# sisl/MADRL

Hardware: AMD Instinct MI355X
Metric: env-steps/sec at fixed batch (PursuitEvade 16x16, 8v30) (higher is better)
Workload: dtype u8/int32 grid state, f32 observations, f64 reward arithmetic; 1 GPU; PursuitEvade 16x16, 8 pursuers / 30 evaders, obs_range 7, rectangle_map, surround, n_catch 2, flatten, local reward, 65536 envs per GPU, horizon 500; envs_per_gpu=65536, envs_total=65536, parallelism=env-sharded x1, streams_per_gpu=2, rccl_ranks=1

## Files before the change

### madrl_amd/csrc/pursuit_wave.hpp

```cpp
#pragma once

#include <type_traits>

#include "common.hpp"

namespace madrl {
namespace pw {

#ifndef MADRL_PW_WAVES
#define MADRL_PW_WAVES 5
#endif
#define MADRL_PW_OCC __attribute__((amdgpu_waves_per_eu(S::OCC, S::OCC)))

constexpr uint32_t SENT = 0xFFFFFFFFu;
constexpr uint32_t CAUGHT = 0x10000u;

struct WaveDev {
    int32_t n_catch, surround, reward_global, sample_maps, n_maps, max_steps, auto_reset;
    int32_t fmap_stride;
    int32_t max_opponents;
    int32_t reverse;
    uint32_t k0, k1, gid_base;
    double catchr, term_pursuit, urgency, cw;
    int64_t n_envs;
    const uint32_t *fmaps;
    const float *vtab;
    const int32_t *pending;
    const uint32_t *cnt_tmpl;
    const uint32_t *slot_tab;
    const double *cw_env;
    const double *catchr_env;
    uint8_t *state;
    uint32_t *flags;
    uint32_t *zmask;
};

struct WaveIO {
    const uint8_t *mask;
    const int32_t *inj_pos;
    const int32_t *inj_map;
    const int32_t *actions;
    const int32_t *inj_eact;
    float *obs;
    float *rew;
    uint8_t *done;
    int32_t *removed;
    int32_t flex;
    int32_t control_evaders;
    const float *obs_prev;
};

__device__ __forceinline__ double sload_f64(const double *p, int64_t index) {
    return ((const __attribute__((address_space(4))) double *)(uint64_t)p)[index];
}

struct KArgs {
    WaveDev d;
    WaveIO io;
};
typedef const __attribute__((address_space(4))) KArgs *KArgsPtr;
__device__ __forceinline__ KArgsPtr cold_args() { return kernargs<KArgs>(); }
__device__ __forceinline__ int32_t pending_count(int64_t env, int k) {
    const int32_t *pend = cold_args()->d.pending;
    return ((const __attribute__((address_space(4))) int32_t *)(uint64_t)pend)[2 * env + k];
}

template <int XS_, int YS_, int P_, int E_, int R_, int FLATTEN_>
struct Shape {
    static constexpr int XS = XS_, YS = YS_, P = P_, E = E_, A = P_ + E_, R = R_, FLATTEN = FLATTEN_;
    static constexpr int OFF = (R - 1) / 2;
    static constexpr int PAD = OFF > 1 ? OFF : 1;
    static constexpr int GW = YS + 2 * PAD;
    static constexpr int GH = XS + 2 * PAD;
    static constexpr int GSZ = (GH * GW + 3) / 4 * 4;
    static constexpr int D = FLATTEN ? 3 * R * R + 1 : 4 * R * R;
    static constexpr int DV = D / 4;
    static constexpr int NQ = P * DV;
    static constexpr int NS = (NQ + 63) / 64;
    static constexpr int MWORDS = 1;
    static constexpr int OCC = NS <= 5 ? MADRL_PW_WAVES : (MADRL_PW_WAVES < 4 ? MADRL_PW_WAVES : 4);
    static constexpr int X_FILL = 3 * GSZ;
    static constexpr int X_SKIP = 3 * GSZ + 1;
    static constexpr int X_ID = 3 * GSZ + 2;
    static constexpr int X_VTAB = (X_ID + P + 3) / 4 * 4;
    static constexpr int NVT = 72;
    static constexpr int X_NEED = X_VTAB + NVT;
    static constexpr int X_OBSV = X_NEED + (XS * YS + 3) / 4;
    static constexpr int LDS_DWORDS = X_OBSV + (P + 3) / 4 * 4;
    static constexpr int NGW = (E + 31) / 32 > 0 ? (E + 31) / 32 : 1;
    static constexpr int NTW = (A + 31) / 32;
    static constexpr int OFF_GONE = (16 + 2 * A + 3) / 4 * 4;
    static constexpr int OFF_TERM = OFF_GONE + 4 * NGW;
    static constexpr int REC_BYTES = (OFF_TERM + 4 * NTW + 15) / 16 * 16;
    static constexpr int REC_DW = REC_BYTES / 4;
    static_assert(REC_DW <= 64, "the whole record must fit one dword per lane");
    static_assert(A <= 64, "one wavefront per env: n_pursuers + n_evaders must fit 64 lanes");
    static_assert(R % 2 == 1, "odd obs_range only (even ranges run on the generic kernel)");
    static_assert(D % 4 == 0, "observation row must be a whole number of float4");
    static_assert(LDS_DWORDS * 4 <= 64 * 1024, "LDS budget");
    static_assert(NS <= 8, "stale-zero mask: one bit per slot in each byte of the lane's mask dword");
    static constexpr bool LIVE = false;
    static constexpr bool TO = false;
    static constexpr bool TABLED = false;
    static constexpr int X_TAB = 0;
};

template <int XS_, int YS_, int P_, int E_, int R_, int FLATTEN_>
struct LShape : Shape<XS_, YS_, P_, E_, R_, FLATTEN_> {
    static constexpr bool LIVE = true;
};
constexpr int NOT_HERE = 0xFF;

template <int XS_, int YS_, int P_, int E_, int R_, int FLATTEN_>
struct TShape : Shape<XS_, YS_, P_, E_, R_, FLATTEN_> {
    static constexpr bool TO = true;
};
template <int XS_, int YS_, int P_, int E_, int R_, int FLATTEN_>
struct TLShape : LShape<XS_, YS_, P_, E_, R_, FLATTEN_> {
    static constexpr bool TO = true;
};

__device__ __forceinline__ double pairwise8(const double *r) {
    return ((r[0] + r[1]) + (r[2] + r[3])) + ((r[4] + r[5]) + (r[6] + r[7]));
}

template <int P>
__device__ __forceinline__ double np_sum_regs(const double (&a)[P]) {
    if constexpr (P < 8) {
        double res = 0.0;
#pragma unroll
        for (int i = 0; i < P; ++i) res += a[i];
        return res;
    } else {
        double r[8];
#pragma unroll
        for (int i = 0; i < 8; ++i) r[i] = a[i];
        constexpr int LIM = P - (P % 8);
#pragma unroll
        for (int i = 8; i < LIM; i += 8) {
#pragma unroll
            for (int k = 0; k < 8; ++k) r[k] += a[i + k];
        }
        double res = pairwise8(r);
#pragma unroll
        for (int i = LIM; i < P; ++i) res += a[i];
        return res;
    }
}

template <int P>
__device__ __forceinline__ double np_sum_first(const double (&a)[P], int n) {
    double res = 0.0;
    if (n < 8) {
#pragma unroll
        for (int i = 0; i < (P < 8 ? P : 7); ++i)
            if (i < n) res += a[i];
        return res;
    }
    if constexpr (P >= 8) {
        double r[8];
#pragma unroll
        for (int i = 0; i < 8; ++i) r[i] = a[i];
        const int lim = n - (n % 8);
#pragma unroll
        for (int i = 8; i + 8 <= P; i += 8) {
            if (i < lim) {
#pragma unroll
                for (int k = 0; k < 8; ++k) r[k] += a[i + k];
            }
        }
        res = pairwise8(r);
#pragma unroll
        for (int i = 8; i < P; ++i)
            if (i >= lim && i < n) res += a[i];
    }
    return res;
}

typedef float v4f_t __attribute__((ext_vector_type(4)));
template <int I, int N, class F>
__device__ __forceinline__ void static_for(F &&f) {
    if constexpr (I < N) {
        f(std::integral_constant<int, I>{});
        static_for<I + 1, N>(f);
    }
}
template <int OFF>
__device__ __forceinline__ void store_slot_masked(const void *base, uint32_t voff, uint32_t v0, uint32_t v1, uint32_t v2, uint32_t v3,
                                                  v4f_t val, uint64_t m0, uint64_t m1, uint64_t m2, uint64_t m3, uint64_t m_nt) {
    uint64_t sv;
    asm volatile("s_mov_b64 %0, exec\n\t"
                 "s_mov_b64 exec, %1\n\tglobal_store_dword %6, %7, %12 offset:%13\n\t"
                 "s_mov_b64 exec, %2\n\tglobal_store_dword %6, %8, %12 offset:%13+4\n\t"
                 "s_mov_b64 exec, %3\n\tglobal_store_dword %6, %9, %12 offset:%13+8\n\t"
                 "s_mov_b64 exec, %4\n\tglobal_store_dword %6, %10, %12 offset:%13+12\n\t"
                 "s_mov_b64 exec, %5\n\tglobal_store_dwordx4 %6, %11, %12 offset:%13 nt\n\t"
                 "s_mov_b64 exec, %0\n\ts_nop 0"
                 : "=&s"(sv) : "s"(m0), "s"(m1), "s"(m2), "s"(m3), "s"(m_nt), "v"(voff), "v"(v0), "v"(v1), "v"(v2), "v"(v3), "v"(val),
                   "s"(base), "n"(OFF));
}
__device__ __forceinline__ uint32_t quad_or(uint32_t v) {
    v |= (uint32_t)__builtin_amdgcn_update_dpp(0, (int)v, 0xB1, 0xF, 0xF, true);
    v |= (uint32_t)__builtin_amdgcn_update_dpp(0, (int)v, 0x4E, 0xF, 0xF, true);
    return v;
}

__device__ __forceinline__ void prefetch3(uint32_t &r0, uint32_t &r1, uint32_t &r2, const void *b0, uint32_t o0, const void *b1, uint32_t o1,
                                          const void *b2, uint32_t o2) {
    asm volatile("s_nop 4\n\tglobal_load_dword %0, %3, %4\n\tglobal_load_dword %1, %5, %6\n\tglobal_load_dword %2, %7, %8"
                 : "=&v"(r0), "=&v"(r1), "=&v"(r2) : "v"(o0), "s"(b0), "v"(o1), "s"(b1), "v"(o2), "s"(b2));
}
template <int N>
__device__ __forceinline__ void prefetch_wait(uint32_t &r0, uint32_t &r1, uint32_t &r2) {
    static_assert(N >= 0 && N < 64, "vmcnt is a 6-bit field");
    asm volatile("s_waitcnt vmcnt(%3)" : "+v"(r0), "+v"(r1), "+v"(r2) : "n"(N) : "memory");
}

template <int LN>
__device__ __forceinline__ void put_lane(uint32_t &w, uint32_t v) {
    const uint32_t sv = (uint32_t)__builtin_amdgcn_readfirstlane((int)v);
    asm("v_writelane_b32 %0, %1, %2" : "+v"(w) : "s"(sv), "n"(LN));
}
template <int LN, int END>
__device__ __forceinline__ void put_zero_from(uint32_t &w) {
    if constexpr (LN < END) {
        put_lane<LN>(w, 0u);
        put_zero_from<LN + 1, END>(w);
    }
}

template <class S, int NT>
struct Fill {
    static constexpr int NEEDW = (S::XS * S::YS + 3) / 4;
    static constexpr int TABW = S::TABLED ? 2 * S::DV : 0;
    static constexpr int J_MAP = (S::GSZ + NT - 1) / NT;
    static constexpr int J_NEED = 2 * J_MAP;
    static constexpr int J_VT = J_NEED + (NEEDW + NT - 1) / NT;
    static constexpr int J_TAB = J_VT + (S::NVT + NT - 1) / NT;
    static constexpr int J_END = J_TAB + (TABW + NT - 1) / NT;
    static constexpr int first(int j) { return j < J_MAP ? 0 : j < J_NEED ? J_MAP : j < J_VT ? J_NEED : j < J_TAB ? J_VT : J_TAB; }
    static constexpr int words(int j) { return j < J_NEED ? S::GSZ : j < J_VT ? NEEDW : j < J_TAB ? S::NVT : TABW; }
};
template <class S, int NT, int J>
__device__ __forceinline__ uint32_t fill_load(uint32_t utid, const uint32_t *cnt, const uint32_t *map, const uint32_t *vtab, const uint32_t *tab) {
    using F = Fill<S, NT>;
    constexpr int t = J - F::first(J), n = F::words(J);
    const uint32_t k = utid + (uint32_t)(NT * t);
    const uint32_t kc = (NT * (t + 1) <= n) ? k : (k < (uint32_t)n ? k : (uint32_t)n - 1u);
    if constexpr (J < F::J_MAP) return cnt[kc];
    else if constexpr (J < F::J_NEED) return map[kc];
    else if constexpr (J < F::J_VT) return map[(uint32_t)S::GSZ + kc];
    else if constexpr (J < F::J_TAB) return vtab[kc];
    else return tab[kc];
}
template <class S, int NT, int J, bool FIRST>
__device__ __forceinline__ void fill_store(uint32_t *L, uint32_t utid, uint32_t v) {
    using F = Fill<S, NT>;
    constexpr int t = J - F::first(J), n = F::words(J);
    const uint32_t k = utid + (uint32_t)(NT * t);
    if ((NT * (t + 1) <= n) || k < (uint32_t)n) {
        if constexpr (J < F::J_MAP) {
            L[S::GSZ + k] = v;
            L[2 * S::GSZ + k] = v;
        } else if constexpr (J < F::J_NEED) L[k] = v;
        else if constexpr (J < F::J_VT) L[S::X_NEED + k] = v;
        else if constexpr (J < F::J_TAB) L[S::X_VTAB + k] = v;
        else L[S::X_TAB + k] = v;
    }
    if constexpr (FIRST && J == F::J_MAP) {
        if (utid == 0u) {
            L[S::X_FILL] = v;
            L[S::X_SKIP] = SENT;
        }
    }
}
template <int N>
__device__ __forceinline__ void staged_wait(uint32_t *a) {
    if constexpr (N >= 8) {
        asm volatile("" : "+v"(a[N - 1]), "+v"(a[N - 2]), "+v"(a[N - 3]), "+v"(a[N - 4]), "+v"(a[N - 5]), "+v"(a[N - 6]), "+v"(a[N - 7]), "+v"(a[N - 8]));
        staged_wait<N - 8>(a);
    } else if constexpr (N >= 4) {
        asm volatile("" : "+v"(a[N - 1]), "+v"(a[N - 2]), "+v"(a[N - 3]), "+v"(a[N - 4]));
        staged_wait<N - 4>(a);
    } else if constexpr (N >= 2) {
        asm volatile("" : "+v"(a[N - 1]), "+v"(a[N - 2]));
        staged_wait<N - 2>(a);
    } else if constexpr (N == 1) {
        asm volatile("" : "+v"(a[0]));
    }
}
template <class S, int NT, int J0, int J1, int CAP, bool FIRST>
__device__ __forceinline__ void fill_trips(uint32_t *L, uint32_t utid, const uint32_t *cnt, const uint32_t *map, const uint32_t *vtab, const uint32_t *tab) {
    if constexpr (J0 < J1) {
        constexpr int JB = J0 + CAP < J1 ? J0 + CAP : J1;
        uint32_t st[JB - J0];
        static_for<J0, JB>([&](auto jc) {
            if constexpr (decltype(jc)::value == JB - 1) __builtin_amdgcn_sched_barrier(0);
            st[decltype(jc)::value - J0] = fill_load<S, NT, decltype(jc)::value>(utid, cnt, map, vtab, tab);
        });
        staged_wait<JB - J0>(st);
        static_for<J0, JB>([&](auto jc) { fill_store<S, NT, decltype(jc)::value, FIRST>(L, utid, st[decltype(jc)::value - J0]); });
        fill_trips<S, NT, JB, J1, CAP, FIRST>(L, utid, cnt, map, vtab, tab);
    }
}
constexpr int FILL_FIRST = 56, FILL_BATCH = 16;

#ifndef MADRL_ABLATE
#define MADRL_ABLATE 0
#endif
#ifndef MADRL_PW_EXP
#define MADRL_PW_EXP 0
#endif

template <class S, int MODE, bool INJECT, bool CTRL = false>
__global__ __launch_bounds__(64) MADRL_PW_OCC void pursuit_wave_kernel(const WaveDev d, const WaveIO io) {
    static_assert(!CTRL || (S::E >= S::P && (MODE == 0 || INJECT)), "evader control: n_evaders >= n_pursuers, flexible instantiation");
    static_assert(!CTRL || !S::LIVE, "evader control has no per-env agent counts");
    static_assert(!S::TO || (MODE == 1 && INJECT && !CTRL), "the two-buffer step: the flexible step kernel only");
    constexpr int P = S::P, E = S::E, A = S::A, GW = S::GW, PAD = S::PAD, GSZ = S::GSZ, NS = S::NS;
    __shared__ __attribute__((aligned(16))) uint32_t L[S::LDS_DWORDS];
    const int lane = threadIdx.x;
    const uint32_t ulane = threadIdx.x;
    const bool is_p = lane < P;
    const int eslot = lane - P;

#if MADRL_PW_EXP & 4
    if (d.n_envs > 0) return;
#endif
    using F = Fill<S, 64>;
    const int n_envs = (int)d.n_envs, stride = (int)gridDim.x;
    if (n_envs <= 0) return;
    auto phys = [&](int e) -> int64_t { return (int64_t)(d.reverse ? n_envs - 1 - e : e); };
    const uint32_t *const vtab_u = reinterpret_cast<const uint32_t *>(d.vtab);
    constexpr int ROOM = FILL_FIRST - 6 * NS - 3;
    constexpr int JF = F::J_END < (ROOM > 4 ? ROOM : 4) ? F::J_END : (ROOM > 4 ? ROOM : 4);
    const uint32_t rec_off = (ulane < (uint32_t)S::REC_DW ? ulane : (uint32_t)S::REC_DW - 1u) * 4u;
    const uint32_t act_off = (ulane < (uint32_t)P ? ulane : (uint32_t)P - 1u) * 4u;
    uint32_t st[JF], sraw[6 * NS];
    static_for<0, JF>([&](auto jc) { st[decltype(jc)::value] = fill_load<S, 64, decltype(jc)::value>(ulane, d.cnt_tmpl, d.fmaps, vtab_u, nullptr); });
#pragma unroll
    for (int k = 0; k < 6 * NS; ++k) sraw[k] = d.slot_tab[64u * k + ulane];
    uint32_t cur_rec, cur_zm;
    int cur_act = 4;
    __builtin_amdgcn_sched_barrier(0);
    {
        const int64_t env0 = phys((int)blockIdx.x < n_envs ? (int)blockIdx.x : n_envs - 1);
        cur_rec = *reinterpret_cast<const uint32_t *>(d.state + env0 * (int64_t)S::REC_BYTES + rec_off);
        if constexpr (MODE == 1) cur_act = *reinterpret_cast<const int *>(reinterpret_cast<const char *>(io.actions + env0 * P) + act_off);
        cur_zm = d.zmask[env0 * 64 + ulane];
    }
    asm volatile("" : "+v"(cur_rec), "+v"(cur_act), "+v"(cur_zm));
    staged_wait<6 * NS>(sraw);
    staged_wait<JF>(st);
    static_for<0, JF>([&](auto jc) { fill_store<S, 64, decltype(jc)::value, true>(L, ulane, st[decltype(jc)::value]); });
    fill_trips<S, 64, JF, F::J_END, FILL_BATCH, true>(L, ulane, d.cnt_tmpl, d.fmaps, vtab_u, nullptr);
    if (lane < P) L[S::X_ID + lane] = __float_as_uint((float)((double)lane / (double)P));
    if (ulane >= (uint32_t)S::REC_DW) cur_rec = 0u;
    if (!is_p) cur_act = 4;
    int s_cst[NS][4];
    int s_rel3[NS];
    int s_src[NS];
#pragma unroll
    for (int s = 0; s < NS; ++s) {
#pragma unroll
        for (int k = 0; k < 4; ++k) s_cst[s][k] = (int)sraw[6 * s + k] * 4;
        s_rel3[s] = (int)sraw[6 * s + 4];
        s_src[s] = (int)sraw[6 * s + 5] * 4;
    }
    int cached_map = 0;
    int cached_np = P;
    const uint8_t *need_tab = reinterpret_cast<const uint8_t *>(&L[S::X_NEED]);
    uint32_t *const layer = &L[is_p ? GSZ : 2 * GSZ];
    const int rec_src0 = (lane >= 4 ? 2 * (lane - 4) : 0) * 4, rec_src1 = rec_src0 + 4;

    auto isP = [&]() { return fresh(lane) < P; };
    auto isE = [&]() { return (unsigned)(fresh(lane) - P) < (unsigned)E; };
    auto isAgent = [&]() { return fresh(lane) < A; };
    auto fetch_rec = [&](int64_t env) -> uint32_t {
        return (fresh(lane) < S::REC_DW) ? uniform_ptr(reinterpret_cast<const uint32_t *>(d.state + env * (int64_t)S::REC_BYTES))[ulane] : 0u;
    };
    auto fetch_act = [&](int64_t env) -> int {
        if constexpr (MODE == 1) return isP() ? uniform_ptr(io.actions + env * P)[ulane] : 4;
        else return 4;
    };
    auto fetch_zm = [&](int64_t env) -> uint32_t { return uniform_ptr(d.zmask + env * 64)[ulane]; };
    wave_sync();
#if MADRL_PW_EXP & 8
    if (d.n_envs > 0) { if (s_cst[0][0] + s_cst[NS - 1][3] + s_rel3[0] + s_src[NS - 1] + (int)cur_rec == 0x12345) io.rew[0] = 1.f; return; }
#endif

    constexpr bool PIPE = (MODE == 1) && !INJECT && !(MADRL_ABLATE & (1 | 8 | 16 | 64));
    constexpr int VM_PER_ENV = 5 * NS + 6;
    static_assert(!PIPE || VM_PER_ENV < 64, "vmcnt range");
    for (int e = blockIdx.x; e < n_envs; e += stride) {
        const int64_t env = phys(e);
        const bool has_next = e + stride < n_envs;
        const int64_t nenv = phys(has_next ? e + stride : e);
        uint32_t nxt_rec = 0, nxt_zm = 0xFFFFFFFFu;
        int nxt_act = 4;
        uint32_t pf_rec, pf_act, pf_zm;
        if constexpr (PIPE) {
            prefetch3(pf_rec, pf_act, pf_zm, d.state + nenv * (int64_t)S::REC_BYTES, rec_off, io.actions + nenv * P, act_off,
                      d.zmask + nenv * 64, ulane * 4u);
        } else {
#if MADRL_ABLATE & 64
            nxt_rec = cur_rec ^ (uint32_t)(fresh(lane) == 0);
            nxt_act = cur_act;
#else
            if (has_next) {
                nxt_rec = fetch_rec(nenv);
                nxt_act = fetch_act(nenv);
                nxt_zm = fetch_zm(nenv);
            }
#endif
        }
        bool skip = false;
        if constexpr (MODE == 0) skip = (io.mask != nullptr && io.mask[env] == 0);
        if (!skip) {
            uint32_t tick = __builtin_amdgcn_readlane(cur_rec, 0);
            int32_t tstep = (int32_t)__builtin_amdgcn_readlane(cur_rec, 1);
            int32_t map_id = (int32_t)__builtin_amdgcn_readlane(cur_rec, 2);
            const uint32_t xyw = (uint32_t)__shfl((int)cur_rec, 4 + (lane >> 1));
            const uint32_t xy = (lane & 1) ? (xyw >> 16) : (xyw & 0xFFFFu);
            int x = (int)(xy & 0xFF), y = (int)(xy >> 8);
            uint64_t gone = (uint32_t)__builtin_amdgcn_readlane(cur_rec, S::OFF_GONE / 4);
            if constexpr (S::NGW > 1) gone |= (uint64_t)(uint32_t)__builtin_amdgcn_readlane(cur_rec, S::OFF_GONE / 4 + 1) << 32;
            uint64_t term = (uint32_t)__builtin_amdgcn_readlane(cur_rec, S::OFF_TERM / 4);
            if constexpr (S::NTW > 1) term |= (uint64_t)(uint32_t)__builtin_amdgcn_readlane(cur_rec, S::OFF_TERM / 4 + 1) << 32;
            const uint32_t gid = d.gid_base + (uint32_t)env;
            const uint32_t k0 = fresh_s(d.k0), k1 = fresh_s(d.k1);
            int np = P, ne = E;
            if constexpr (S::LIVE) {
                const bool here = x != NOT_HERE;
                np = __popcll(__builtin_amdgcn_ballot_w64(isP() && here));
                ne = __popcll(__builtin_amdgcn_ballot_w64(isE() && here));
                if (!here) {
                    x = 0;
                    y = 0;
                }
            }
            auto isLP = [&]() {
                if constexpr (S::LIVE) return fresh(lane) < np;
                else return isP();
            };
            bool do_reset = (MODE == 0);
            uint32_t done_bits = 0;
            float rew_out = 0.0f;
            int n_removed = 0;
            bool alive = isLP() || (isE() && !((gone >> eslot) & 1ull));
            int cell = (x + PAD) * GW + y + PAD;

            auto load_map = [&](int mid) {
                if (cached_map == mid) return;
                const KArgsPtr ka = cold_args();
                fill_trips<S, 64, F::J_MAP, F::J_VT, FILL_BATCH, false>(L, ulane, nullptr, ka->d.fmaps + (int64_t)mid * ka->d.fmap_stride, nullptr, nullptr);
                cached_map = mid;
                wave_sync();
            };
            load_map(map_id);

            if constexpr (MODE == 1) {
                const bool e_alive = alive && !isP();
                if (e_alive) atomicAdd(&layer[cell], 1u);
                wave_sync();
                int kpre = 0;
                if (isP()) {
                    const int dxm = (x > 0) ? GW : 0, dxp = (x < S::XS - 1) ? GW : 0;
                    const int dym = (y > 0) ? 1 : 0, dyp = (y < S::YS - 1) ? 1 : 0;
                    const uint32_t *ec = &L[2 * GSZ];
                    kpre = (int)(ec[cell - dxm] + ec[cell + dxp] + ec[cell + dyp] + ec[cell - dym]);
                }
                wave_sync();
                if (e_alive) atomicSub(&layer[cell], 1u);
                const int kidx = __popcll((~gone) & ((1ull << (eslot & 63)) - 1ull));
                int act = cur_act;
                bool injected = false;
                if constexpr (CTRL) {
                    const int from_k = __builtin_amdgcn_ds_bpermute((kidx < P ? kidx : 0) * 4, cur_act);
                    injected = io.inj_eact != nullptr;
                    int pact;
                    if (injected) pact = isP() ? io.inj_eact[env * P + lane] : 4;
                    else pact = (int)__umulhi(philox4x32_10(gid, tick, (uint32_t)lane, TAG_PURSUER_ACT, k0, k1).x, 5u);
                    act = isP() ? pact : (kidx < P ? from_k : 4);
                    injected = true;
                } else if constexpr (INJECT) {
                    injected = io.inj_eact != nullptr;
                    if (injected && e_alive) act = io.inj_eact[env * E + kidx];
                }
                if (!injected) {
#if MADRL_ABLATE & 4
                    u32x4 r; r.x = (gid * 2654435761u + tick * 40503u + (uint32_t)kidx * 2246822519u) ^ k0 ^ k1;
#else
                    const u32x4 r = philox4x32_10(gid, tick, (uint32_t)kidx, TAG_EVADER_ACT, k0, k1);
#endif
                    if (!isP()) act = (int)__umulhi(r.x, 5u);
                }
                const int dcell = (act == 0 ? -GW : 0) + (act == 1 ? GW : 0) + (act == 2 ? 1 : 0) + (act == 3 ? -1 : 0);
                const bool tflag = (term >> lane) & 1ull;
                const bool in_building = L[cell] != 0u;
                const bool target_free = L[cell + dcell] == 0u;
                const bool newterm = alive && !tflag && in_building;
                if (alive && !tflag && !in_building && target_free) {
                    cell += dcell;
                    x += (act == 1) - (act == 0);
                    y += (act == 2) - (act == 3);
                }
                term |= __ballot(newterm);
                if (alive) atomicAdd(&layer[cell], 1u);
                wave_sync();
                bool caught = false;
                if (e_alive) {
                    const uint32_t *pc = &L[GSZ];
                    if (d.surround) {
                        const uint32_t n0 = pc[cell - GW], n1 = pc[cell + GW], n2 = pc[cell + 1], n3 = pc[cell - 1];
                        const int cnt = (int)(n0 - 1u < SENT - 1u) + (int)(n1 - 1u < SENT - 1u) +
                                        (int)(n2 - 1u < SENT - 1u) + (int)(n3 - 1u < SENT - 1u);
                        caught = cnt == (int)need_tab[x * S::YS + y];
                    } else {
                        caught = (int)pc[cell] >= d.n_catch;
                    }
                    if (caught) atomicAdd(&layer[cell], CAUGHT);
                }
                const uint64_t caught_mask = __ballot(caught) >> P;
                gone |= caught_mask;
                wave_sync();
                double r = 0.0;
                if (isLP()) {
                    const uint32_t *ec = &L[2 * GSZ];
                    bool sur;
                    if (d.surround) {
                        const uint32_t n0 = ec[cell - GW], n1 = ec[cell + GW], n2 = ec[cell + 1], n3 = ec[cell - 1];
                        sur = ((n0 != SENT) & (n0 >= CAUGHT)) | ((n1 != SENT) & (n1 >= CAUGHT)) |
                              ((n2 != SENT) & (n2 >= CAUGHT)) | ((n3 != SENT) & (n3 >= CAUGHT));
                    } else {
                        sur = ec[cell] >= CAUGHT;
                    }
                    double catchr = d.catchr;
                    if constexpr (INJECT) { if (d.catchr_env != nullptr) catchr = sload_f64(d.catchr_env, env); }
                    r = catchr * (double)kpre;
                    r += d.term_pursuit * (sur ? 1.0 : 0.0);
                    r += d.urgency;
                }
                if (d.reward_global) {
                    double all[P];
#pragma unroll
                    for (int k = 0; k < P; ++k) all[k] = __shfl(r, k);
                    if constexpr (S::LIVE) r = isLP() ? np_sum_first<P>(all, np) / (double)np : 0.0;
                    else r = np_sum_regs<P>(all) / (double)P;
                }
                tick += 1;
                tstep += 1;
                constexpr uint64_t all_e = (1ull << E) - 1ull;
                if ((gone & all_e) == all_e) done_bits |= 1u;
                if (d.max_steps > 0 && tstep >= d.max_steps) done_bits |= 2u;
                do_reset = d.auto_reset && done_bits != 0;
                rew_out = (float)r;
                n_removed = __popcll(caught_mask);
            }

            if constexpr (!PIPE) asm volatile("" : "+v"(nxt_rec), "+v"(nxt_act), "+v"(nxt_zm));
            uint32_t zm = cur_zm;

            const int npass = (MODE == 1 && do_reset) ? 2 : 1;
            for (int pass = 0; pass < npass; ++pass) {
                if (do_reset && pass == npass - 1) {
                    gone = 0ull;
                    term = 0ull;
                    const KArgsPtr ka = cold_args();
                    const double cw = ka->d.cw_env != nullptr ? sload_f64(ka->d.cw_env, env) : ka->d.cw;
                    const int max_opponents = ka->d.max_opponents;
                    bool inj_map = false, inj_pos = false;
                    if constexpr (MODE == 0) {
                        inj_map = io.inj_map != nullptr;
                        inj_pos = io.inj_pos != nullptr;
                    }
                    if (inj_map) {
                        map_id = __builtin_amdgcn_readfirstlane(io.inj_map[env]);
                    } else if (ka->d.sample_maps) {
                        const u32x4 rm = philox4x32_10(gid, tick, 0u, TAG_RESET_ENV, k0, k1);
                        map_id = (int)__umulhi(rm.x, (uint32_t)ka->d.n_maps);
                    }
                    load_map(map_id);
                    const u32x4 rw = philox4x32_10(gid, tick, 1u, TAG_RESET_ENV, k0, k1);
                    const double sx = u53(rw.x, rw.y) * (1.0 - cw);
                    const double sy = u53(rw.z, rw.w) * (1.0 - cw);
                    const int xlb = (int)(S::XS * sx), xub = (int)(S::XS * (sx + cw));
                    const int ylb = (int)(S::YS * sy), yub = (int)(S::YS * (sy + cw));
                    int n_create = E;
                    if constexpr (S::LIVE) {
                        np = min(max(pending_count(env, 0), 1), P);
                        ne = min(max(pending_count(env, 1), 0), E);
                        n_create = ne;
                    }
                    if (max_opponents > 0 && !inj_pos) {
                        const u32x4 r3 = philox4x32_10(gid, tick, 2u, TAG_RESET_ENV, k0, k1);
                        n_create = min(1 + (int)__umulhi(r3.x, (uint32_t)(max_opponents - 1)), S::LIVE ? ne : E);
                    }
                    bool exists = false;
                    if (isAgent()) {
                        if constexpr (S::LIVE) exists = isLP() || (!isP() && eslot < n_create);
                        else exists = isP() || eslot < n_create;
                        if (inj_pos) {
                            x = io.inj_pos[(env * A + lane) * 2];
                            y = io.inj_pos[(env * A + lane) * 2 + 1];
                            if (!isP() && x < 0) exists = false;
                        } else {
                            for (uint32_t att = 0; att < 1024u; ++att) {
                                const uint32_t aidx = S::LIVE ? (uint32_t)(isP() ? lane : np + eslot) : (uint32_t)lane;
                                const u32x4 rp = philox4x32_10(gid, tick, aidx, TAG_RESET_POS | (att << 8), k0, k1);
                                x = xlb + (int)__umulhi(rp.x, (uint32_t)(xub - xlb));
                                y = ylb + (int)__umulhi(rp.y, (uint32_t)(yub - ylb));
                                if (L[(x + PAD) * GW + y + PAD] == 0u) break;
                            }
                        }
                        if (exists) {
                            cell = (x + PAD) * GW + y + PAD;
                            atomicAdd(&layer[cell], 1u);
                        } else {
                            x = 0;
                            y = 0;
                        }
                    }
                    gone = __ballot(isE() && !exists) >> P;
                    alive = exists;
                    tick += 1;
                    tstep = 0;
                    wave_sync();
                }
                if constexpr (S::LIVE) {
                    if (np != cached_np) {
                        if (lane < P) L[S::X_ID + lane] = __float_as_uint((float)((double)lane / (double)np));
                        cached_np = np;
                        wave_sync();
                    }
                }
                uint32_t cnt = 0;
                if (alive) cnt = layer[cell] & 0xFFFFu;
                wave_sync();
                if (alive) layer[cell] = L[S::X_VTAB + cnt];
                wave_sync();
#if MADRL_ABLATE & 8
                if (d.n_envs < 0)
#endif
                {
                    int origin = isP() ? ((x - S::OFF + PAD) * GW + (y - S::OFF + PAD)) * 4 : 0;
                    int n_rows = P;
                    if constexpr (CTRL) {
                        const uint64_t obsv = ~gone & ((1ull << P) - 1ull);
                        n_rows = __popcll(obsv);
                        const bool is_obs = isE() && eslot < P && ((obsv >> (eslot & 63)) & 1ull);
                        if (is_obs) L[S::X_OBSV + __popcll(obsv & ((1ull << (eslot & 63)) - 1ull))] = (uint32_t)(((x - S::OFF + PAD) * GW + (y - S::OFF + PAD)) * 4);
                        wave_sync();
                        origin = (isP() && lane < n_rows) ? (int)L[S::X_OBSV + lane] : 0;
                    }
                    if constexpr (S::LIVE) n_rows = np;
                    const char *orow_u = (const char *)uniform_ptr(io.obs + env * (int64_t)(P * S::D));
                    asm volatile("s_nop 4" : "+s"(orow_u));
                    const uint32_t voff = ulane * 16u;
                    [[maybe_unused]] const auto prow_g = uniform_ptr(S::TO ? io.obs_prev + env * (int64_t)(P * S::D) : io.obs);
                    [[maybe_unused]] const auto orow_g = uniform_ptr(io.obs + env * (int64_t)(P * S::D));
                    const char *Lb = reinterpret_cast<const char *>(L);
                    auto cell_at = [&](int off) -> uint32_t { return *reinterpret_cast<const uint32_t *>(Lb + off); };
                    uint32_t acc = 0u;
                    [[maybe_unused]] uint32_t to_need[S::TO ? NS : 1], to_bits[S::TO ? NS : 1];
                    static_for<0, NS>([&](auto sc) {
                        constexpr int s = decltype(sc)::value;
                        const int base = __builtin_amdgcn_ds_bpermute(s_src[s], origin);
                        const uint32_t v0 = cell_at(base + s_cst[s][0]);
                        const uint32_t v1 = cell_at(base + s_cst[s][1]);
                        const uint32_t v2 = cell_at(base + s_cst[s][2]);
                        const uint32_t v3 = cell_at((int)__umul24((uint32_t)base, (uint32_t)s_rel3[s]) + s_cst[s][3]);
                        const uint32_t top = __builtin_amdgcn_perm(v1, v0, 0x0C0C0703u) | __builtin_amdgcn_perm(v3, v2, 0x07030C0Cu);
                        const uint32_t out4 = (top >> 7) & 0x01010101u;
                        const uint32_t nz4 = ((top >> 5) | (top >> 6)) & 0x01010101u;
                        const uint32_t old4 = (zm >> (NS - 1 - s)) & 0x01010101u;
                        const uint32_t dirty = out4 & old4;
                        if constexpr (S::TO) {
                            if (pass == 0) {
                                bool row_live = true;
                                if constexpr (S::LIVE) row_live = (s_src[s] >> 2) < n_rows;
                                const bool in_row = (64 * (s + 1) <= S::NQ) ? true : (fresh(lane) + 64 * s < S::NQ);
                                const uint32_t need4 = in_row ? (row_live ? dirty : 0x01010101u) : 0u;
                                to_need[s] = need4;
                                to_bits[s] = ~need4 & ~out4 & nz4;
                                return;
                            }
                        }
                        bool valid = (64 * (s + 1) <= S::NQ) ? true : (fresh(lane) + 64 * s < S::NQ);
                        if constexpr (CTRL || S::LIVE) {
                            const bool row_live = (s_src[s] >> 2) < n_rows;
                            acc = (acc << 1) | (row_live ? ((out4 & old4) | (~out4 & nz4)) : old4);
                            valid = valid && row_live;
                        } else {
                            acc = (acc << 1) | ((out4 & old4) | (~out4 & nz4));
                        }
                        bool clean = dirty == 0u;
#if MADRL_ABLATE & 1
                        valid = d.n_envs < 0;
#endif
#if MADRL_ABLATE & 2
                        clean = true;
#endif
                        const uint32_t st = valid ? (clean ? 0u : dirty) : 0x80000000u;
#if MADRL_ABLATE & 32
                        {
                            uint32_t burn = acc;
                            asm volatile("v_xor_b32 %0, %0, %1\n v_xor_b32 %0, %0, %1\n v_xor_b32 %0, %0, %1\n v_xor_b32 %0, %0, %1\n v_xor_b32 %0, %0, %1\n"
                                         "v_xor_b32 %0, %0, %1\n v_xor_b32 %0, %0, %1\n v_xor_b32 %0, %0, %1\n v_xor_b32 %0, %0, %1\n v_xor_b32 %0, %0, %1\n"
                                         "v_xor_b32 %0, %0, %1\n v_xor_b32 %0, %0, %1\n v_xor_b32 %0, %0, %1\n v_xor_b32 %0, %0, %1\n v_xor_b32 %0, %0, %1\n"
                                         "v_xor_b32 %0, %0, %1\n v_xor_b32 %0, %0, %1\n v_xor_b32 %0, %0, %1\n v_xor_b32 %0, %0, %1\n v_xor_b32 %0, %0, %1"
                                         : "+v"(burn) : "v"(v0));
                            acc = burn;
                        }
#endif
#if MADRL_ABLATE & 128
                        {
                            uint32_t sburn = fresh_s(0u);
                            asm volatile("s_add_u32 %0, %0, 1\n s_add_u32 %0, %0, 1\n s_add_u32 %0, %0, 1\n s_add_u32 %0, %0, 1\n s_add_u32 %0, %0, 1\n"
                                         "s_add_u32 %0, %0, 1\n s_add_u32 %0, %0, 1\n s_add_u32 %0, %0, 1\n s_add_u32 %0, %0, 1\n s_add_u32 %0, %0, 1\n"
                                         "s_add_u32 %0, %0, 1\n s_add_u32 %0, %0, 1\n s_add_u32 %0, %0, 1\n s_add_u32 %0, %0, 1\n s_add_u32 %0, %0, 1\n"
                                         "s_add_u32 %0, %0, 1\n s_add_u32 %0, %0, 1\n s_add_u32 %0, %0, 1\n s_add_u32 %0, %0, 1\n s_add_u32 %0, %0, 1"
                                         : "+s"(sburn) : : "scc");
                        }
#endif
                        const void *sb = orow_u + 4096 * (s / 4);
                        const uint32_t lim = (uint32_t)fresh((st - 1u < 0x01010101u) ? (int)SENT : 0);
                        const uint32_t grp = quad_or(st == 0u ? (out4 ^ 0x01010101u) : 0u);
                        const uint32_t nt = (uint32_t)fresh(st == 0u ? (int)grp : 0);
                        const v4f_t val = {__uint_as_float((uint32_t)max((int)v0, 0)), __uint_as_float((uint32_t)max((int)v1, 0)),
                                           __uint_as_float((uint32_t)max((int)v2, 0)), __uint_as_float((uint32_t)max((int)v3, 0))};
                        store_slot_masked<1024 * (s % 4)>(sb, voff, v0, v1, v2, v3, val, __builtin_amdgcn_ballot_w64(v0 < lim),
                                                          __builtin_amdgcn_ballot_w64(v1 < lim), __builtin_amdgcn_ballot_w64(v2 < lim),
                                                          __builtin_amdgcn_ballot_w64(v3 < lim), __builtin_amdgcn_ballot_w64(nt != 0u));
                    });
                    if constexpr (S::TO) {
                        if (pass == 0) {
                            typedef uint32_t v4u_t __attribute__((ext_vector_type(4)));
                            typedef __attribute__((address_space(1))) v4u_t gv4u_t;
                            typedef __attribute__((address_space(1))) v4f_t gv4f_t;
                            constexpr int TG = NS <= 5 ? NS : 4;
                            auto emit = [&](auto sc, const v4u_t oldv) {
                                constexpr int s = decltype(sc)::value;
                                const int base = __builtin_amdgcn_ds_bpermute(s_src[s], origin);
                                const uint32_t need4 = to_need[s];
                                uint32_t w0 = (uint32_t)max((int)cell_at(base + s_cst[s][0]), 0);
                                uint32_t w1 = (uint32_t)max((int)cell_at(base + s_cst[s][1]), 0);
                                uint32_t w2 = (uint32_t)max((int)cell_at(base + s_cst[s][2]), 0);
                                uint32_t w3 = (uint32_t)max((int)cell_at((int)__umul24((uint32_t)base, (uint32_t)s_rel3[s]) + s_cst[s][3]), 0);
                                if (need4 & 0x00000001u) w0 = oldv.x;
                                if (need4 & 0x00000100u) w1 = oldv.y;
                                if (need4 & 0x00010000u) w2 = oldv.z;
                                if (need4 & 0x01000000u) w3 = oldv.w;
                                const uint32_t oldnz = (oldv.x != 0u ? 0x00000001u : 0u) | (oldv.y != 0u ? 0x00000100u : 0u) |
                                                       (oldv.z != 0u ? 0x00010000u : 0u) | (oldv.w != 0u ? 0x01000000u : 0u);
                                acc = (acc << 1) | to_bits[s] | (need4 & oldnz);
                                const bool in_row = (64 * (s + 1) <= S::NQ) ? true : (fresh(lane) + 64 * s < S::NQ);
                                if (in_row) {
                                    const v4f_t wv = {__uint_as_float(w0), __uint_as_float(w1), __uint_as_float(w2), __uint_as_float(w3)};
                                    __builtin_nontemporal_store(wv, reinterpret_cast<gv4f_t *>(orow_g) + (64u * s + ulane));
                                }
                            };
                            static_for<0, (NS + TG - 1) / TG>([&](auto gc) {
                                constexpr int g0 = decltype(gc)::value * TG, g1 = g0 + TG < NS ? g0 + TG : NS;
                                uint32_t any = 0u;
#pragma unroll
                                for (int s = g0; s < g1; ++s) any |= to_need[s];
                                if (__builtin_amdgcn_ballot_w64(any != 0u) != 0ull) {
                                    v4u_t old[TG];
#pragma unroll
                                    for (int s = g0; s < g1; ++s) {
                                        old[s - g0] = v4u_t{0u, 0u, 0u, 0u};
                                        if (to_need[s] != 0u) old[s - g0] = reinterpret_cast<const gv4u_t *>(prow_g)[64u * s + ulane];
                                    }
                                    static_for<g0, g1>([&](auto sc) { emit(sc, old[decltype(sc)::value - g0]); });
                                } else {
                                    static_for<g0, g1>([&](auto sc) { emit(sc, v4u_t{0u, 0u, 0u, 0u}); });
                                }
                            });
                        }
                    }
                    zm = acc;
                }
                wave_sync();
                if (alive) layer[cell] = 0u;
                wave_sync();
            }
#if MADRL_ABLATE & 16
            if (d.n_envs < 0)
#endif
            if constexpr (MODE == 1) {
                if (isP()) uniform_ptr(io.rew + env * P)[ulane] = rew_out;
                if (fresh(lane) == 0) {
                    io.done[env] = (uint8_t)done_bits;
                    io.removed[env] = n_removed;
                    cold_args()->d.flags[env] = done_flag_word(done_bits);
                }
            }
            {
                int myxy = x | (y << 8);
                if constexpr (S::LIVE) {
                    if (!(isP() ? isLP() : eslot < ne)) myxy = NOT_HERE | (NOT_HERE << 8);
                }
                const uint32_t lo = (uint32_t)__builtin_amdgcn_ds_bpermute(rec_src0, myxy);
                const uint32_t hi = (uint32_t)__builtin_amdgcn_ds_bpermute(rec_src1, myxy);
                uint32_t w = (lo & 0xFFFFu) | (hi << 16);
                put_lane<0>(w, tick);
                put_lane<1>(w, (uint32_t)tstep);
                put_lane<2>(w, (uint32_t)map_id);
                put_lane<3>(w, 0u);
                put_lane<S::OFF_GONE / 4>(w, (uint32_t)gone);
                if constexpr (S::NGW > 1) put_lane<S::OFF_GONE / 4 + 1>(w, (uint32_t)(gone >> 32));
                put_lane<S::OFF_TERM / 4>(w, (uint32_t)term);
                if constexpr (S::NTW > 1) put_lane<S::OFF_TERM / 4 + 1>(w, (uint32_t)(term >> 32));
                put_zero_from<S::OFF_TERM / 4 + S::NTW, S::REC_DW>(w);
#if MADRL_ABLATE & 16
                if (d.n_envs < 0)
#endif
                if (fresh(lane) < S::REC_DW)
                    uniform_ptr(reinterpret_cast<uint32_t *>(d.state + env * (int64_t)S::REC_BYTES))[ulane] = w;
#if MADRL_ABLATE & 16
                if (d.n_envs < 0)
#endif
                uniform_ptr(d.zmask + env * 64)[ulane] = zm;
            }
        }
        if constexpr (PIPE) {
            prefetch_wait<VM_PER_ENV>(pf_rec, pf_act, pf_zm);
            nxt_rec = (fresh(lane) < S::REC_DW) ? pf_rec : 0u;
            nxt_act = (int)pf_act;
            nxt_zm = pf_zm;
        }
        cur_rec = nxt_rec;
        cur_act = nxt_act;
        cur_zm = nxt_zm;
    }
}

template <class S>
void wave_to_launch(const WaveDev &d, const WaveIO &io, int64_t blocks, hipStream_t s);

}
}
```

Baseline: 1.158 billion env-steps/s.

## Pin kernel args in SGPRs, batch action draws, fold conv lookup, rotate slot reads

Loads loop-invariant kernel arguments once and pins them in scalar registers so they are not re-fetched from the kernarg segment. The random action draw and the neighbour/target LDS reads move before the first barrier. The post-move cell-to-vtab conversion is computed early and reused in the first pass. Observation slot reads are software-pipelined one slot ahead. These changes aim to cut scalar reloads, LDS latency and barriers, at the cost of more live registers, which may reduce occupancy.

```diff
diff --git a/madrl_amd/csrc/pursuit_wave.hpp b/madrl_amd/csrc/pursuit_wave.hpp
--- a/madrl_amd/csrc/pursuit_wave.hpp
+++ b/madrl_amd/csrc/pursuit_wave.hpp
@@ -102,6 +102,7 @@
     static constexpr bool LIVE = false;
     static constexpr bool TO = false;
     static constexpr bool TABLED = false;
+    static constexpr bool ROTATE = true;
     static constexpr int X_TAB = 0;
 };
 
@@ -311,6 +312,24 @@
 #ifndef MADRL_PW_EXP
 #define MADRL_PW_EXP 0
 #endif
+constexpr bool CH_ARGS = !(MADRL_PW_EXP & 16), CH_ROT = !(MADRL_PW_EXP & 32), CH_DRAW = !(MADRL_PW_EXP & 64), CH_CONV = !(MADRL_PW_EXP & 128);
+
+template <class T>
+__device__ __forceinline__ T pinned(T v) {
+    static_assert(sizeof(T) == 4 || sizeof(T) == 8, "one SGPR or an SGPR pair");
+    if constexpr (sizeof(T) == 4) {
+        uint32_t b;
+        __builtin_memcpy(&b, &v, 4);
+        asm volatile("" : "+s"(b));
+        __builtin_memcpy(&v, &b, 4);
+    } else {
+        uint64_t b;
+        __builtin_memcpy(&b, &v, 8);
+        asm volatile("" : "+s"(b));
+        __builtin_memcpy(&v, &b, 8);
+    }
+    return v;
+}
 
 template <class S, int MODE, bool INJECT, bool CTRL = false>
 __global__ __launch_bounds__(64) MADRL_PW_OCC void pursuit_wave_kernel(const WaveDev d, const WaveIO io) {
@@ -328,7 +347,7 @@
     if (d.n_envs > 0) return;
 #endif
     using F = Fill<S, 64>;
-    const int n_envs = (int)d.n_envs, stride = (int)gridDim.x;
+    const int n_envs = (int)d.n_envs;
     if (n_envs <= 0) return;
     auto phys = [&](int e) -> int64_t { return (int64_t)(d.reverse ? n_envs - 1 - e : e); };
     const uint32_t *const vtab_u = reinterpret_cast<const uint32_t *>(d.vtab);
@@ -392,6 +411,15 @@
     constexpr bool PIPE = (MODE == 1) && !INJECT && !(MADRL_ABLATE & (1 | 8 | 16 | 64));
     constexpr int VM_PER_ENV = 5 * NS + 6;
     static_assert(!PIPE || VM_PER_ENV < 64, "vmcnt range");
+    constexpr bool PIN = CH_ARGS && MODE == 1 && !CTRL;
+    const int stride = PIN ? pinned((int)gridDim.x) : (int)gridDim.x;
+    const int32_t *const actions = PIN ? pinned(io.actions) : io.actions;
+    const double urgency = PIN ? pinned(d.urgency) : d.urgency, catchr0 = PIN ? pinned(d.catchr) : d.catchr;
+    const double term_pursuit = PIN ? pinned(d.term_pursuit) : d.term_pursuit;
+    const int surround = PIN ? pinned(d.surround) : d.surround, n_catch = PIN ? pinned(d.n_catch) : d.n_catch;
+    const int reward_global = PIN ? pinned(d.reward_global) : d.reward_global;
+    const int max_steps = PIN ? pinned(d.max_steps) : d.max_steps, auto_reset = PIN ? pinned(d.auto_reset) : d.auto_reset;
+    const auto flag_words = (__attribute__((address_space(1))) uint32_t *)(PIN ? pinned(d.flags) : nullptr);
     for (int e = blockIdx.x; e < n_envs; e += stride) {
         const int64_t env = phys(e);
         const bool has_next = e + stride < n_envs;
@@ -400,7 +428,7 @@
         int nxt_act = 4;
         uint32_t pf_rec, pf_act, pf_zm;
         if constexpr (PIPE) {
-            prefetch3(pf_rec, pf_act, pf_zm, d.state + nenv * (int64_t)S::REC_BYTES, rec_off, io.actions + nenv * P, act_off,
+            prefetch3(pf_rec, pf_act, pf_zm, d.state + nenv * (int64_t)S::REC_BYTES, rec_off, actions + nenv * P, act_off,
                       d.zmask + nenv * 64, ulane * 4u);
         } else {
 #if MADRL_ABLATE & 64
@@ -449,6 +477,8 @@
             int n_removed = 0;
             bool alive = isLP() || (isE() && !((gone >> eslot) & 1ull));
             int cell = (x + PAD) * GW + y + PAD;
+            constexpr bool BATCH = CH_DRAW && MODE == 1 && !(S::TO && S::LIVE), FOLD = CH_CONV && MODE == 1, SAFE_CELL = BATCH || FOLD;
+            if constexpr (SAFE_CELL) { if (!isAgent()) cell = PAD * GW + PAD; }
 
             auto load_map = [&](int mid) {
                 if (cached_map == mid) return;
@@ -459,12 +489,50 @@
             };
             load_map(map_id);
 
+            [[maybe_unused]] uint32_t conv = 0u;
             if constexpr (MODE == 1) {
                 const bool e_alive = alive && !isP();
+                const int kidx = __popcll((~gone) & ((1ull << (eslot & 63)) - 1ull));
+                int act = cur_act;
+                auto draw = [&]() {
+                    bool injected = false;
+                    if constexpr (CTRL) {
+                        const int from_k = __builtin_amdgcn_ds_bpermute((kidx < P ? kidx : 0) * 4, cur_act);
+                        injected = io.inj_eact != nullptr;
+                        int pact;
+                        if (injected) pact = isP() ? io.inj_eact[env * P + lane] : 4;
+                        else pact = (int)__umulhi(philox4x32_10(gid, tick, (uint32_t)lane, TAG_PURSUER_ACT, k0, k1).x, 5u);
+                        act = isP() ? pact : (kidx < P ? from_k : 4);
+                        injected = true;
+                    } else if constexpr (INJECT) {
+                        injected = io.inj_eact != nullptr;
+                        if (injected && e_alive) act = io.inj_eact[env * E + kidx];
+                    }
+                    if (!injected) {
+#if MADRL_ABLATE & 4
+                        u32x4 r; r.x = (gid * 2654435761u + tick * 40503u + (uint32_t)kidx * 2246822519u) ^ k0 ^ k1;
+#else
+                        const u32x4 r = philox4x32_10(gid, tick, (uint32_t)kidx, TAG_EVADER_ACT, k0, k1);
+#endif
+                        if (!isP()) act = (int)__umulhi(r.x, 5u);
+                    }
+                };
+                auto step_of = [&](int a) { return (a == 0 ? -GW : 0) + (a == 1 ? GW : 0) + (a == 2 ? 1 : 0) + (a == 3 ? -1 : 0); };
                 if (e_alive) atomicAdd(&layer[cell], 1u);
                 wave_sync();
-                int kpre = 0;
-                if (isP()) {
+                int kpre = 0, dcell = 0;
+                uint32_t m_here = 0u, m_to = 0u;
+                if constexpr (BATCH) {
+                    draw();
+                    dcell = step_of(act);
+                    const int dxm = (x > 0) ? GW : 0, dxp = (x < S::XS - 1) ? GW : 0;
+                    const int dym = (y > 0) ? 1 : 0, dyp = (y < S::YS - 1) ? 1 : 0;
+                    const uint32_t *ec = &L[2 * GSZ];
+                    const uint32_t c0 = ec[cell - dxm], c1 = ec[cell + dxp], c2 = ec[cell + dyp], c3 = ec[cell - dym];
+                    m_here = L[cell];
+                    m_to = L[cell + dcell];
+                    kpre = (int)(c0 + c1 + c2 + c3);
+                } else if (isP()) {
                     const int dxm = (x > 0) ? GW : 0, dxp = (x < S::XS - 1) ? GW : 0;
                     const int dym = (y > 0) ? 1 : 0, dyp = (y < S::YS - 1) ? 1 : 0;
                     const uint32_t *ec = &L[2 * GSZ];
@@ -472,33 +540,15 @@
                 }
                 wave_sync();
                 if (e_alive) atomicSub(&layer[cell], 1u);
-                const int kidx = __popcll((~gone) & ((1ull << (eslot & 63)) - 1ull));
-                int act = cur_act;
-                bool injected = false;
-                if constexpr (CTRL) {
-                    const int from_k = __builtin_amdgcn_ds_bpermute((kidx < P ? kidx : 0) * 4, cur_act);
-                    injected = io.inj_eact != nullptr;
-                    int pact;
-                    if (injected) pact = isP() ? io.inj_eact[env * P + lane] : 4;
-                    else pact = (int)__umulhi(philox4x32_10(gid, tick, (uint32_t)lane, TAG_PURSUER_ACT, k0, k1).x, 5u);
-                    act = isP() ? pact : (kidx < P ? from_k : 4);
-                    injected = true;
-                } else if constexpr (INJECT) {
-                    injected = io.inj_eact != nullptr;
-                    if (injected && e_alive) act = io.inj_eact[env * E + kidx];
-                }
-                if (!injected) {
-#if MADRL_ABLATE & 4
-                    u32x4 r; r.x = (gid * 2654435761u + tick * 40503u + (uint32_t)kidx * 2246822519u) ^ k0 ^ k1;
-#else
-                    const u32x4 r = philox4x32_10(gid, tick, (uint32_t)kidx, TAG_EVADER_ACT, k0, k1);
-#endif
-                    if (!isP()) act = (int)__umulhi(r.x, 5u);
-                }
-                const int dcell = (act == 0 ? -GW : 0) + (act == 1 ? GW : 0) + (act == 2 ? 1 : 0) + (act == 3 ? -1 : 0);
+                if constexpr (!BATCH) {
+                    draw();
+                    dcell = step_of(act);
+                    m_here = L[cell];
+                    m_to = L[cell + dcell];
+                }
                 const bool tflag = (term >> lane) & 1ull;
-                const bool in_building = L[cell] != 0u;
-                const bool target_free = L[cell + dcell] == 0u;
+                const bool in_building = m_here != 0u;
+                const bool target_free = m_to == 0u;
                 const bool newterm = alive && !tflag && in_building;
                 if (alive && !tflag && !in_building && target_free) {
                     cell += dcell;
@@ -508,16 +558,17 @@
                 term |= __ballot(newterm);
                 if (alive) atomicAdd(&layer[cell], 1u);
                 wave_sync();
+                if constexpr (FOLD) conv = layer[cell];
                 bool caught = false;
                 if (e_alive) {
                     const uint32_t *pc = &L[GSZ];
-                    if (d.surround) {
+                    if (surround) {
                         const uint32_t n0 = pc[cell - GW], n1 = pc[cell + GW], n2 = pc[cell + 1], n3 = pc[cell - 1];
                         const int cnt = (int)(n0 - 1u < SENT - 1u) + (int)(n1 - 1u < SENT - 1u) +
                                         (int)(n2 - 1u < SENT - 1u) + (int)(n3 - 1u < SENT - 1u);
                         caught = cnt == (int)need_tab[x * S::YS + y];
                     } else {
-                        caught = (int)pc[cell] >= d.n_catch;
+                        caught = (int)pc[cell] >= n_catch;
                     }
                     if (caught) atomicAdd(&layer[cell], CAUGHT);
                 }
@@ -525,23 +576,24 @@
                 gone |= caught_mask;
                 wave_sync();
                 double r = 0.0;
+                if constexpr (FOLD) conv = L[S::X_VTAB + (conv & 0xFFFFu)];
                 if (isLP()) {
                     const uint32_t *ec = &L[2 * GSZ];
                     bool sur;
-                    if (d.surround) {
+                    if (surround) {
                         const uint32_t n0 = ec[cell - GW], n1 = ec[cell + GW], n2 = ec[cell + 1], n3 = ec[cell - 1];
                         sur = ((n0 != SENT) & (n0 >= CAUGHT)) | ((n1 != SENT) & (n1 >= CAUGHT)) |
                               ((n2 != SENT) & (n2 >= CAUGHT)) | ((n3 != SENT) & (n3 >= CAUGHT));
                     } else {
                         sur = ec[cell] >= CAUGHT;
                     }
-                    double catchr = d.catchr;
+                    double catchr = catchr0;
                     if constexpr (INJECT) { if (d.catchr_env != nullptr) catchr = sload_f64(d.catchr_env, env); }
                     r = catchr * (double)kpre;
-                    r += d.term_pursuit * (sur ? 1.0 : 0.0);
-                    r += d.urgency;
-                }
-                if (d.reward_global) {
+                    r += term_pursuit * (sur ? 1.0 : 0.0);
+                    r += urgency;
+                }
+                if (reward_global) {
                     double all[P];
 #pragma unroll
                     for (int k = 0; k < P; ++k) all[k] = __shfl(r, k);
@@ -552,8 +604,8 @@
                 tstep += 1;
                 constexpr uint64_t all_e = (1ull << E) - 1ull;
                 if ((gone & all_e) == all_e) done_bits |= 1u;
-                if (d.max_steps > 0 && tstep >= d.max_steps) done_bits |= 2u;
-                do_reset = d.auto_reset && done_bits != 0;
+                if (max_steps > 0 && tstep >= max_steps) done_bits |= 2u;
+                do_reset = auto_reset && done_bits != 0;
                 rew_out = (float)r;
                 n_removed = __popcll(caught_mask);
             }
@@ -634,10 +686,15 @@
                         wave_sync();
                     }
                 }
-                uint32_t cnt = 0;
-                if (alive) cnt = layer[cell] & 0xFFFFu;
-                wave_sync();
-                if (alive) layer[cell] = L[S::X_VTAB + cnt];
+                if (FOLD && pass == 0) {
+                    wave_sync();
+                    if (alive) layer[cell] = conv;
+                } else {
+                    uint32_t cnt = 0;
+                    if (alive) cnt = layer[cell] & 0xFFFFu;
+                    wave_sync();
+                    if (alive) layer[cell] = L[S::X_VTAB + cnt];
+                }
                 wave_sync();
 #if MADRL_ABLATE & 8
                 if (d.n_envs < 0)
@@ -663,13 +720,22 @@
                     auto cell_at = [&](int off) -> uint32_t { return *reinterpret_cast<const uint32_t *>(Lb + off); };
                     uint32_t acc = 0u;
                     [[maybe_unused]] uint32_t to_need[S::TO ? NS : 1], to_bits[S::TO ? NS : 1];
+                    constexpr bool ROT = CH_ROT && S::ROTATE;
+                    uint32_t cv[NS][4];
+                    auto read_slot = [&](auto sc) {
+                        constexpr int s = decltype(sc)::value;
+                        const int base = __builtin_amdgcn_ds_bpermute(s_src[s], origin);
+                        cv[s][0] = cell_at(base + s_cst[s][0]);
+                        cv[s][1] = cell_at(base + s_cst[s][1]);
+                        cv[s][2] = cell_at(base + s_cst[s][2]);
+                        cv[s][3] = cell_at((int)__umul24((uint32_t)base, (uint32_t)s_rel3[s]) + s_cst[s][3]);
+                    };
+                    if constexpr (ROT) read_slot(std::integral_constant<int, 0>{});
                     static_for<0, NS>([&](auto sc) {
                         constexpr int s = decltype(sc)::value;
-                        const int base = __builtin_amdgcn_ds_bpermute(s_src[s], origin);
-                        const uint32_t v0 = cell_at(base + s_cst[s][0]);
-                        const uint32_t v1 = cell_at(base + s_cst[s][1]);
-                        const uint32_t v2 = cell_at(base + s_cst[s][2]);
-                        const uint32_t v3 = cell_at((int)__umul24((uint32_t)base, (uint32_t)s_rel3[s]) + s_cst[s][3]);
+                        if constexpr (!ROT) read_slot(sc);
+                        else if constexpr (s + 1 < NS) read_slot(std::integral_constant<int, s + 1>{});
+                        const uint32_t v0 = cv[s][0], v1 = cv[s][1], v2 = cv[s][2], v3 = cv[s][3];
                         const uint32_t top = __builtin_amdgcn_perm(v1, v0, 0x0C0C0703u) | __builtin_amdgcn_perm(v3, v2, 0x07030C0Cu);
                         const uint32_t out4 = (top >> 7) & 0x01010101u;
                         const uint32_t nz4 = ((top >> 5) | (top >> 6)) & 0x01010101u;
@@ -793,7 +859,8 @@
                 if (fresh(lane) == 0) {
                     io.done[env] = (uint8_t)done_bits;
                     io.removed[env] = n_removed;
-                    cold_args()->d.flags[env] = done_flag_word(done_bits);
+                    if constexpr (PIN) flag_words[env] = done_flag_word(done_bits);
+                    else cold_args()->d.flags[env] = done_flag_word(done_bits);
                 }
             }
             {
```

Result: no change. 1.162 billion env-steps/s, median of 3 (+0.3%).
